# frankyeh/UNet-Studio

Hardware: AMD Instinct MI355X
Metric: voxels/sec 3D U-Net train step @128^3 bf16 (higher is better)
Workload: dtype bf16

## Files before the change

unet-studio_amd/csrc/kernels_direct.hip:

```cpp
#include "device_util.h"

namespace unet {

__global__ void k_pack_conv_w(const float* __restrict__ w, float* __restrict__ wf, float* __restrict__ wd, int Cin, int Cout,
                              int k3, int CoutP, int CinP) {
    int64_t i = (int64_t)blockIdx.x * blockDim.x + threadIdx.x;
    int64_t nf = (int64_t)k3 * Cin * CoutP, nd = (int64_t)k3 * Cout * CinP;
    if (i < nf) {
        int co = (int)(i % CoutP); int64_t r = i / CoutP;
        int ci = (int)(r % Cin); int t = (int)(r / Cin);
        wf[i] = co < Cout ? w[((int64_t)co * Cin + ci) * k3 + t] : 0.f;
    }
    if (i < nd) {
        int ci = (int)(i % CinP); int64_t r = i / CinP;
        int co = (int)(r % Cout); int t = (int)(r / Cout);
        wd[i] = ci < Cin ? w[((int64_t)co * Cin + ci) * k3 + t] : 0.f;
    }
}
__global__ void k_pack_convt_w(const float* __restrict__ w, float* __restrict__ wf, float* __restrict__ wd, int Cin, int Cout,
                               int CoutP, int CinP) {
    int64_t i = (int64_t)blockIdx.x * blockDim.x + threadIdx.x;
    int64_t nf = (int64_t)8 * Cin * CoutP, nd = (int64_t)8 * Cout * CinP;
    if (i < nf) {
        int co = (int)(i % CoutP); int64_t r = i / CoutP;
// ... 621 lines not shown
    small_wgrad_epilogue<NACC>(acc, nchunk, sm, a.slab + (int64_t)blockIdx.x * (O + Cout), [=](int ch, int i) {
        if (i < CO * 16) { int c = i / 16, k = i % 16; return c < Cout ? c * Cin + ch * 16 + k : -1; }
        int c = i - CO * 16;
        return (ch == 0 && c < Cout) ? O + c : -1;
    });
}

constexpr int FIRST_TY = 8;
template <typename T> __global__ void __launch_bounds__(256) k_wgrad_first(WgradRegArgs a) {
    extern __shared__ float sm[];
    constexpr int NACC = 27 * 4 + 4;
    const ConvGeom& g = a.g;
    const int nchunk = 1 << a.lc, chunk = threadIdx.x & (nchunk - 1), co0 = chunk * 4;
    const int W4 = g.W >> 2, WP = (g.W + 2 + 3) & ~3;
    const int ytiles = (g.H + FIRST_TY - 1) / FIRST_TY, tiles = g.D * ytiles;
    const int nin = 3 * (FIRST_TY + 2) * WP;
    const int items = (FIRST_TY * W4) << a.lc;
    const T* dy = (const T*)a.dy;
    float acc[NACC];
#pragma unroll
    for (int i = 0; i < NACC; ++i) acc[i] = 0.f;
    for (int tile = blockIdx.x; tile < tiles; tile += gridDim.x) {
        const int z = tile / ytiles, y0 = (tile % ytiles) * FIRST_TY;
        __syncthreads();
        for (int i = threadIdx.x; i < nin; i += 256) {
            const int px = i % WP, r = i / WP, ry = r % (FIRST_TY + 2), rz = r / (FIRST_TY + 2);
            const int iz = z + rz - 1, iy = y0 + ry - 1, ix = px - 1;
            float v = 0.f;
            if (iz >= 0 && iz < g.D && iy >= 0 && iy < g.H && ix >= 0 && ix < g.W) v = view_ld<T>(a.src, ((int64_t)iz * g.H + iy) * g.W + ix, 0);
            sm[i] = v;
        }
        __syncthreads();
        for (int it = threadIdx.x; it < items; it += 256) {
            const int run = it >> a.lc, ty = run / W4, x0 = (run % W4) * 4;
            if (y0 + ty >= g.H) continue;
            float in[3][3][6], ds[4][4];
#pragma unroll
            for (int kz = 0; kz < 3; ++kz)
#pragma unroll
                for (int ky = 0; ky < 3; ++ky) {
                    const float* row = sm + (kz * (FIRST_TY + 2) + ty + ky) * WP + x0;
                    const float4 q = *(const float4*)row;
                    const float2 q2 = *(const float2*)(row + 4);
                    in[kz][ky][0] = q.x; in[kz][ky][1] = q.y; in[kz][ky][2] = q.z; in[kz][ky][3] = q.w;
                    in[kz][ky][4] = q2.x; in[kz][ky][5] = q2.y;
                }
            const int64_t vox = ((int64_t)z * g.H + y0 + ty) * g.W + x0;
#pragma unroll
            for (int u = 0; u < 4; ++u) {
                if constexpr (sizeof(T) == 2) {
                    const uint2 r = *(const uint2*)((const bf16*)dy + (vox + u) * g.Cout + co0);
                    ds[u][0] = __uint_as_float(r.x << 16); ds[u][1] = __uint_as_float(r.x & 0xffff0000u);
                    ds[u][2] = __uint_as_float(r.y << 16); ds[u][3] = __uint_as_float(r.y & 0xffff0000u);
                } else {
                    const float4 r = *(const float4*)((const float*)dy + (vox + u) * g.Cout + co0);
                    ds[u][0] = r.x; ds[u][1] = r.y; ds[u][2] = r.z; ds[u][3] = r.w;
                }
            }
#pragma unroll
            for (int kz = 0; kz < 3; ++kz)
#pragma unroll
                for (int ky = 0; ky < 3; ++ky)
#pragma unroll
                    for (int kx = 0; kx < 3; ++kx)
#pragma unroll
                        for (int u = 0; u < 4; ++u)
#pragma unroll
                            for (int c = 0; c < 4; ++c)
                                acc[((kz * 3 + ky) * 3 + kx) * 4 + c] = fmaf(in[kz][ky][u + kx], ds[u][c], acc[((kz * 3 + ky) * 3 + kx) * 4 + c]);
#pragma unroll
            for (int u = 0; u < 4; ++u)
#pragma unroll
                for (int c = 0; c < 4; ++c) acc[108 + c] += ds[u][c];
        }
    }
    __syncthreads();
    const int Cout = g.Cout, O = 27 * Cout;
    small_wgrad_epilogue<NACC>(acc, nchunk, sm, a.slab + (int64_t)blockIdx.x * (O + Cout), [=](int ch, int i) {
        if (i < 108) return (ch * 4 + i % 4) * 27 + i / 4;
        return O + ch * 4 + (i - 108);
    });
}

template <typename T> __device__ __forceinline__ void load_chunk16(const SrcDesc& src, bool plain, int64_t v, int c0, bool ok, float (&x)[16],
                                                                  const float* ss = nullptr, int Cin = 0) {
    if constexpr (sizeof(T) == 2) {
        if (plain || ss) {
            uint4 r0 = make_uint4(0, 0, 0, 0), r1 = r0;
            if (ok) {
                const uint4* q = (const uint4*)((const bf16*)src.ptr + v * src.C + c0);
                r0 = q[0]; r1 = q[1];
            }
            const unsigned w[8] = {r0.x, r0.y, r0.z, r0.w, r1.x, r1.y, r1.z, r1.w};
#pragma unroll
            for (int k = 0; k < 8; ++k) { x[2 * k] = __uint_as_float(w[k] << 16); x[2 * k + 1] = __uint_as_float(w[k] & 0xffff0000u); }
            if (!plain) {
#pragma unroll
                for (int k4 = 0; k4 < 4; ++k4) {
                    const float4 sc = *(const float4*)(ss + c0 + 4 * k4), sh = *(const float4*)(ss + Cin + c0 + 4 * k4);
                    x[4 * k4] = act_f(x[4 * k4] * sc.x + sh.x, src.act); x[4 * k4 + 1] = act_f(x[4 * k4 + 1] * sc.y + sh.y, src.act);
                    x[4 * k4 + 2] = act_f(x[4 * k4 + 2] * sc.z + sh.z, src.act); x[4 * k4 + 3] = act_f(x[4 * k4 + 3] * sc.w + sh.w, src.act);
                }
                if (!ok) {
#pragma unroll
                    for (int k = 0; k < 16; ++k) x[k] = 0.f;
                }
            }
            return;
        }
    }
#pragma unroll
    for (int k = 0; k < 16; ++k) x[k] = ok ? view_ld<T>(src, v, c0 + k) : 0.f;
}
template <typename T> __device__ __forceinline__ const float* stage_view(const SrcDesc& src, float* sm_after_filter, int Cin) {
    if (sizeof(T) != 2 || !src.scale) return nullptr;
    for (int i = threadIdx.x; i < Cin; i += 256) { sm_after_filter[i] = src.scale[i]; sm_after_filter[Cin + i] = src.shift[i]; }
    return sm_after_filter;
}

struct HeadArgs {
    SrcDesc src;
    const float* w;
    const float* bias;
    int Cin, Cout, lc;
    int64_t S;
    void* y;
    float* out;
    const float* dy_planes;
    const void* dy_cl;
    DstGrad dst;
    float* slab;
};

template <typename T, int CO> __global__ void __launch_bounds__(256) k_head_fwd(HeadArgs a) {
    extern __shared__ float sm[];
    for (int i = threadIdx.x; i < CO * a.Cin; i += 256) sm[i] = i < a.Cout * a.Cin ? a.w[i] : 0.f;
    const float* ss = stage_view<T>(a.src, sm + CO * a.Cin, a.Cin);
    __syncthreads();
    const int nchunk = 1 << a.lc, chunk = threadIdx.x & (nchunk - 1), c0 = chunk * 16;
    const int64_t vstride = ((int64_t)gridDim.x * 256) >> a.lc;
    const bool plain = !a.src.scale && a.src.act == 0;
    float b[CO];
#pragma unroll
    for (int c = 0; c < CO; ++c) b[c] = (a.bias && c < a.Cout) ? a.bias[c] : 0.f;
    for (int64_t v0 = ((int64_t)blockIdx.x * 256 + threadIdx.x) >> a.lc; v0 < ((a.S + 63) & ~(int64_t)63); v0 += vstride) {
        const bool ok = v0 < a.S;
        float x[16], o[CO];
        load_chunk16<T>(a.src, plain, v0, c0, ok, x, ss, a.Cin);
#pragma unroll
        for (int c = 0; c < CO; ++c) {
            const float4* wr = (const float4*)(sm + c * a.Cin + c0);
            float r = 0.f;
#pragma unroll
            for (int k4 = 0; k4 < 4; ++k4) {
                const float4 w4 = wr[k4];
                r = fmaf(x[4 * k4], w4.x, r); r = fmaf(x[4 * k4 + 1], w4.y, r); r = fmaf(x[4 * k4 + 2], w4.z, r); r = fmaf(x[4 * k4 + 3], w4.w, r);
            }
            for (int m = 1; m < nchunk; m <<= 1) r += __shfl_xor(r, m);
            o[c] = r + b[c];
        }
        if (ok && chunk == 0) {
#pragma unroll
            for (int c = 0; c < CO; ++c) {
                if (c < a.Cout) {
                    if (a.out) a.out[(int64_t)c * a.S + v0] = o[c];
                    if (a.y) st<T>((T*)a.y, v0 * a.Cout + c, o[c]);
                }
            }
        }
    }
}

template <typename T, int CO> __global__ void __launch_bounds__(256) k_head_bwd(HeadArgs a) {
    extern __shared__ float sm[];
    constexpr int NACC = CO * 16 + CO;
    for (int i = threadIdx.x; i < CO * a.Cin; i += 256) sm[i] = i < a.Cout * a.Cin ? a.w[i] : 0.f;
    const float* ss = stage_view<T>(a.src, sm + CO * a.Cin, a.Cin);
    __syncthreads();
    const int nchunk = 1 << a.lc, chunk = threadIdx.x & (nchunk - 1), c0 = chunk * 16;
    const int64_t vstride = ((int64_t)gridDim.x * 256) >> a.lc;
    const bool plain = !a.src.scale && a.src.act == 0;
    float acc[NACC];
#pragma unroll
    for (int i = 0; i < NACC; ++i) acc[i] = 0.f;
    auto fetch = [&](int64_t v, float (&xo)[16], float (&dout)[CO]) {
        load_chunk16<T>(a.src, plain, v, c0, true, xo, ss, a.Cin);
#pragma unroll
        for (int c = 0; c < CO; ++c) {
            dout[c] = 0.f;
            if (c < a.Cout) dout[c] = a.dy_planes ? a.dy_planes[(int64_t)c * a.S + v] : ld<T>((const T*)a.dy_cl, v * a.Cout + c);
        }
    };
    float xn[16], dn[CO];
    int64_t v0 = ((int64_t)blockIdx.x * 256 + threadIdx.x) >> a.lc;
    if (v0 < a.S) fetch(v0, xn, dn);
    for (; v0 < a.S; v0 += vstride) {
        float x[16], d[CO];
#pragma unroll
        for (int k = 0; k < 16; ++k) x[k] = xn[k];
#pragma unroll
        for (int c = 0; c < CO; ++c) d[c] = dn[c];
        if (v0 + vstride < a.S) fetch(v0 + vstride, xn, dn);
        if (a.slab) {
#pragma unroll
            for (int c = 0; c < CO; ++c) {
#pragma unroll
                for (int k = 0; k < 16; ++k) acc[c * 16 + k] = fmaf(d[c], x[k], acc[c * 16 + k]);
                acc[CO * 16 + c] += d[c];
            }
        }
        if (a.dst.ptr) {
            float g[16];
#pragma unroll
            for (int k = 0; k < 16; ++k) g[k] = 0.f;
#pragma unroll
            for (int c = 0; c < CO; ++c) {
                const float4* wr = (const float4*)(sm + c * a.Cin + c0);
#pragma unroll
                for (int k4 = 0; k4 < 4; ++k4) {
                    const float4 w4 = wr[k4];
                    g[4 * k4] = fmaf(d[c], w4.x, g[4 * k4]); g[4 * k4 + 1] = fmaf(d[c], w4.y, g[4 * k4 + 1]);
                    g[4 * k4 + 2] = fmaf(d[c], w4.z, g[4 * k4 + 2]); g[4 * k4 + 3] = fmaf(d[c], w4.w, g[4 * k4 + 3]);
                }
            }
            if constexpr (sizeof(T) == 2) {
                uint4* q = (uint4*)((bf16*)a.dst.ptr + v0 * a.dst.C + c0);
                if (a.dst.accumulate) {
                    const uint4 r0 = q[0], r1 = q[1];
                    const unsigned w[8] = {r0.x, r0.y, r0.z, r0.w, r1.x, r1.y, r1.z, r1.w};
#pragma unroll
                    for (int k = 0; k < 8; ++k) { g[2 * k] += __uint_as_float(w[k] << 16); g[2 * k + 1] += __uint_as_float(w[k] & 0xffff0000u); }
                }
                unsigned pk[8];
#pragma unroll
                for (int k = 0; k < 8; ++k) {
                    const bf16 lo = __float2bfloat16(g[2 * k]), hi = __float2bfloat16(g[2 * k + 1]);
                    pk[k] = (unsigned)__builtin_bit_cast(unsigned short, lo) | ((unsigned)__builtin_bit_cast(unsigned short, hi) << 16);
                }
                q[0] = make_uint4(pk[0], pk[1], pk[2], pk[3]); q[1] = make_uint4(pk[4], pk[5], pk[6], pk[7]);
            } else {
                float* q = (float*)a.dst.ptr + v0 * a.dst.C + c0;
#pragma unroll
                for (int k = 0; k < 16; ++k) q[k] = a.dst.accumulate ? q[k] + g[k] : g[k];
            }
        }
    }
    if (a.slab) {
        __syncthreads();
        const int Cin = a.Cin, Cout = a.Cout, O = Cin * Cout;
        small_wgrad_epilogue<NACC>(acc, nchunk, sm, a.slab + (int64_t)blockIdx.x * (O + Cout), [=](int ch, int i) {
            if (i < CO * 16) { int c = i / 16, k = i % 16; return c < Cout ? c * Cin + ch * 16 + k : -1; }
            int c = i - CO * 16;
            return (ch == 0 && c < Cout) ? O + c : -1;
        });
    }
}

static int ilog2_exact(int v) { int l = 0; while ((1 << l) < v) ++l; return (1 << l) == v ? l : -1; }
static bool wgrad_head_ok(const ConvGeom& g, int nsrc) {
    return nsrc == 1 && g.ks == 1 && g.stride == 1 && g.Cout <= 8 && g.Cin % 16 == 0 && ilog2_exact(g.Cin / 16) >= 0 && g.Cin <= 256;
}
static bool wgrad_first_ok(const ConvGeom& g, int nsrc) {
    return nsrc == 1 && g.ks == 3 && g.stride == 1 && g.Cin == 1 && g.Cout % 4 == 0 && ilog2_exact(g.Cout / 4) >= 0 && g.Cout <= 64 &&
           g.W % 4 == 0 && g.W <= 256;
}
static int wgrad_reg_blocks(int64_t items4) { int64_t nb = (items4 + 1023) / 1024; return nb < 1 ? 1 : (nb > 512 ? 512 : (int)nb); }
static bool wgrad_rows_ok(const ConvGeom& g) {
    int k3 = g.ks * g.ks * g.ks;
    int WI = (g.Wo - 1) * g.stride + g.ks;
    size_t lds = ((size_t)g.ks * g.ks * WI * g.Cin + (size_t)g.Wo * g.Cout) * 4;
    return (int64_t)k3 * g.Cin * g.Cout <= 1024 && lds <= 48 * 1024;
}

static int wgrad_small_blocks(const ConvGeom& g) { int rows = g.Do * g.Ho; return rows < 1024 ? rows : 1024; }
bool wgrad_small_supported(const ConvGeom& g, int nsrc) { return wgrad_head_ok(g, nsrc) || wgrad_first_ok(g, nsrc) || wgrad_rows_ok(g); }
size_t wgrad_small_scratch_bytes(const ConvGeom& g) {
    int k3 = g.ks * g.ks * g.ks;
    int64_t So = (int64_t)g.Do * g.Ho * g.Wo;
    size_t O = (size_t)k3 * g.Cin * g.Cout;
    size_t rows = (size_t)wgrad_small_blocks(g) * O * 4 + bias_grad_scratch_bytes(g.Cout, So) + 256;
    size_t regs = (size_t)512 * (O + g.Cout) * 4 + 256;
    return rows > regs ? rows : regs;
}
void launch_conv_wgrad_small(int dtype, const ConvGeom& g, const SrcDesc* src, int nsrc, const void* dy, float* dw, float* db,
                             void* scratch, hipStream_t s) {
    const int k3 = g.ks * g.ks * g.ks;
    const int64_t O = (int64_t)k3 * g.Cin * g.Cout;
    const bool head = wgrad_head_ok(g, nsrc), first = !head && wgrad_first_ok(g, nsrc);
    if (head || first) {
        WgradRegArgs a;
        a.g = g; a.src = src[0]; a.dy = dy; a.slab = (float*)scratch;
        const int64_t S = (int64_t)g.D * g.H * g.W;
        int nb;
        if (head) {
            a.lc = ilog2_exact(g.Cin / 16);
            nb = wgrad_reg_blocks((S << a.lc) * 4);
            const int CO = g.Cout <= 2 ? 2 : g.Cout <= 4 ? 4 : g.Cout <= 6 ? 6 : 8;
            const size_t lds = small_wgrad_lds_bytes(CO * 17, 1 << a.lc);
            switch (CO) {
                case 2: UNET_DISPATCH(dtype, (k_wgrad_head<T, 2><<<nb, 256, lds, s>>>(a))); break;
                case 4: UNET_DISPATCH(dtype, (k_wgrad_head<T, 4><<<nb, 256, lds, s>>>(a))); break;
                case 6: UNET_DISPATCH(dtype, (k_wgrad_head<T, 6><<<nb, 256, lds, s>>>(a))); break;
                default: UNET_DISPATCH(dtype, (k_wgrad_head<T, 8><<<nb, 256, lds, s>>>(a))); break;
            }
        } else {
            a.lc = ilog2_exact(g.Cout / 4);
            const int tiles = g.D * ((g.H + FIRST_TY - 1) / FIRST_TY);
            nb = tiles < 512 ? tiles : 512;
            const size_t l0 = (size_t)3 * (FIRST_TY + 2) * ((g.W + 5) & ~3) * 4, l1 = small_wgrad_lds_bytes(112, 1 << a.lc);
            const size_t lds = l0 > l1 ? l0 : l1;
            UNET_DISPATCH(dtype, (k_wgrad_first<T><<<nb, 256, lds, s>>>(a)));
        }
        slab_reduce2(a.slab, nb, O + g.Cout, dw, O, db, s);
        return;
    }
    WgradSmallArgs a;
    a.g = g; a.nsrc = nsrc; a.src[0] = src[0]; if (nsrc > 1) a.src[1] = src[1];
    a.dy = dy; a.slab = (float*)scratch;
    int nb = wgrad_small_blocks(g);
    int WI = (g.Wo - 1) * g.stride + g.ks;
    size_t lds = ((size_t)g.ks * g.ks * WI * g.Cin + (size_t)g.Wo * g.Cout) * 4;
    UNET_DISPATCH(dtype, (k_wgrad_small<T><<<nb, 256, lds, s>>>(a)));
    slab_reduce(a.slab, nb, O, dw, s);
    if (db) launch_bias_grad(dtype, dy, g.Cout, (int64_t)g.Do * g.Ho * g.Wo, db, (float*)scratch + (size_t)nb * O, s);
}

bool head_supported(const ConvGeom& g, int nsrc) { return wgrad_head_ok(g, nsrc); }
size_t head_bwd_scratch_bytes(const ConvGeom& g) { return (size_t)512 * ((size_t)g.Cin * g.Cout + g.Cout) * 4 + 256; }
template <typename T> static void head_launch(bool bwd, int CO, int nb, size_t lds, const HeadArgs& a, hipStream_t s) {
    switch (CO) {
        case 2: if (bwd) k_head_bwd<T, 2><<<nb, 256, lds, s>>>(a); else k_head_fwd<T, 2><<<nb, 256, lds, s>>>(a); break;
        case 4: if (bwd) k_head_bwd<T, 4><<<nb, 256, lds, s>>>(a); else k_head_fwd<T, 4><<<nb, 256, lds, s>>>(a); break;
        case 6: if (bwd) k_head_bwd<T, 6><<<nb, 256, lds, s>>>(a); else k_head_fwd<T, 6><<<nb, 256, lds, s>>>(a); break;
        default: if (bwd) k_head_bwd<T, 8><<<nb, 256, lds, s>>>(a); else k_head_fwd<T, 8><<<nb, 256, lds, s>>>(a); break;
    }
}
static int head_co(int Cout) { return Cout <= 2 ? 2 : Cout <= 4 ? 4 : Cout <= 6 ? 6 : 8; }
void launch_head_fwd(int dtype, const ConvGeom& g, const SrcDesc& src, const float* w, const float* bias, void* y, float* out_ncdhw,
                     hipStream_t s) {
    HeadArgs a = {};
    a.src = src; a.w = w; a.bias = bias; a.Cin = g.Cin; a.Cout = g.Cout; a.lc = ilog2_exact(g.Cin / 16);
    a.S = (int64_t)g.D * g.H * g.W; a.y = y; a.out = out_ncdhw;
    const int CO = head_co(g.Cout);
    int64_t items = ((a.S + 63) & ~(int64_t)63) << a.lc;
    int64_t nb = (items + 255) / 256;
    if (nb > 2048) nb = 2048;
    UNET_DISPATCH(dtype, (head_launch<T>(false, CO, (int)nb, (size_t)(CO + 2) * g.Cin * 4, a, s)));
}
void launch_head_bwd(int dtype, const ConvGeom& g, const SrcDesc& src, const float* dy_ncdhw, const void* dy_cl, const float* w,
                     DstGrad dst, float* dw, float* db, void* scratch, hipStream_t s, bool defer_reduce) {
    HeadArgs a = {};
    a.src = src; a.w = w; a.Cin = g.Cin; a.Cout = g.Cout; a.lc = ilog2_exact(g.Cin / 16);
    a.S = (int64_t)g.D * g.H * g.W; a.dy_planes = dy_ncdhw; a.dy_cl = dy_cl; a.dst = dst;
    a.slab = dw ? (float*)scratch : nullptr;
    const int CO = head_co(g.Cout);
    const int nb = wgrad_reg_blocks((a.S << a.lc) * 4);
    const size_t l0 = (size_t)(CO + 2) * g.Cin * 4, l1 = small_wgrad_lds_bytes(CO * 17, 1 << a.lc);
    UNET_DISPATCH(dtype, (head_launch<T>(true, CO, nb, l0 > l1 ? l0 : l1, a, s)));
    if (dw && !defer_reduce) slab_reduce2(a.slab, nb, (int64_t)g.Cin * g.Cout + g.Cout, dw, (int64_t)g.Cin * g.Cout, db, s);
}
void launch_head_bwd_reduce(const ConvGeom& g, float* dw, float* db, const void* scratch, hipStream_t s) {
    const int lc = ilog2_exact(g.Cin / 16);
    const int nb = wgrad_reg_blocks((((int64_t)g.D * g.H * g.W) << lc) * 4);
    slab_reduce2((const float*)scratch, nb, (int64_t)g.Cin * g.Cout + g.Cout, dw, (int64_t)g.Cin * g.Cout, db, s);
}

}
```

unet-studio_amd/csrc/kernels_elem.hip:

```cpp
#include "device_util.h"
#include "sgd_update.h"

namespace unet {

template <typename T> __global__ void k_pack_input(const float* __restrict__ x, T* __restrict__ y, int C, int64_t S) {
    int64_t i = (int64_t)blockIdx.x * 256 + threadIdx.x;
    if (i >= S * C) return;
    int c = (int)(i % C); int64_t v = i / C;
    st<T>(y, i, x[(int64_t)c * S + v]);
}
void launch_pack_input(int dtype, const float* x, void* y, int C, int64_t S, hipStream_t s) {
    UNET_DISPATCH(dtype, (k_pack_input<T><<<cdiv64(S * C, 256), 256, 0, s>>>(x, (T*)y, C, S)));
}

template <typename T> __global__ void k_export(SrcDesc src, float* __restrict__ y, int64_t S) {
    int64_t i = (int64_t)blockIdx.x * 256 + threadIdx.x;
    if (i >= S * src.C) return;
    int c = (int)(i / S); int64_t v = i % S;
    y[i] = view_ld<T>(src, v, c);
}
void launch_export(int dtype, SrcDesc src, float* y, int64_t S, hipStream_t s) {
    UNET_DISPATCH(dtype, (k_export<T><<<cdiv64(S * src.C, 256), 256, 0, s>>>(src, y, S)));
}
void launch_unpack_ncdhw(int dtype, const void* g, float* out, int C, int64_t S, hipStream_t s) {
// ... 717 lines not shown
        bool valid = t < C;
        if (!valid) continue;
        int tt = k ? (int)(t - k + 1 > 0 ? t - k + 1 : 0) : (int)t;
        VoxelLogits L = make_vl(logits, S, v, k);
        float mx = -INFINITY;
        for (int c = 0; c < oc; ++c) mx = fmaxf(mx, L.get(c));
        float sum = 0.f;
        for (int c = 0; c < oc; ++c) sum += __expf(L.get(c) - mx);
        float inv = 1.f / sum, psq = 0.f, pt = 0.f;
        for (int c = 0; c < oc; ++c) {
            float p = clamp_p(__expf(L.get(c) - mx) * inv);
            psq = fmaf(p, p, psq);
            if (c == tt) pt = p;
            if (c >= 1) atomicAdd(&sh[3 + oc + c], p + (c == tt ? 1.f : 0.f));
        }
        if (tt >= 1) atomicAdd(&sh[3 + tt], pt);
        ce += -(L.get(tt) - mx - __logf(sum));
        mse += psq - 2.f * pt + 1.f;
        nv += 1.f;
    }
    atomicAdd(&sh[0], ce); atomicAdd(&sh[1], mse); atomicAdd(&sh[2], nv);
    __syncthreads();
    for (int i = threadIdx.x; i < np; i += 256) partial[(int64_t)blockIdx.x * np + i] = sh[i];
}
template <int OCMAX>
__global__ void __launch_bounds__(256) k_loss_partial_reg(const float* __restrict__ logits, const int64_t* __restrict__ target, int C,
                                                          int64_t S, int k, float* __restrict__ partial) {
    constexpr int RS = 3 + 2 * OCMAX + 1;
    __shared__ float red[4 * RS];
    const int oc = k ? C - k + 1 : C, np = 3 + 2 * oc;
    float ce = 0.f, mse = 0.f, nv = 0.f, inter[OCMAX], card[OCMAX];
#pragma unroll
    for (int c = 0; c < OCMAX; ++c) { inter[c] = 0.f; card[c] = 0.f; }
    for (int64_t v = (int64_t)blockIdx.x * 256 + threadIdx.x; v < S; v += (int64_t)gridDim.x * 256) {
        int64_t t = target[v];
        if (!(t < C)) continue;
        int tt = k ? (int)(t - k + 1 > 0 ? t - k + 1 : 0) : (int)t;
        VoxelLogits L = make_vl(logits, S, v, k);
        float lg[OCMAX], mx = -INFINITY;
#pragma unroll
        for (int c = 0; c < OCMAX; ++c) { lg[c] = c < oc ? L.get(c) : -INFINITY; mx = fmaxf(mx, lg[c]); }
        float sum = 0.f;
#pragma unroll
        for (int c = 0; c < OCMAX; ++c) { lg[c] = c < oc ? __expf(lg[c] - mx) : 0.f; sum += lg[c]; }
        float inv = 1.f / sum, psq = 0.f, pt = 0.f, lt = 0.f;
#pragma unroll
        for (int c = 0; c < OCMAX; ++c) {
            if (c < oc) {
                float p = clamp_p(lg[c] * inv);
                psq = fmaf(p, p, psq);
                bool hit = c == tt;
                if (hit) { pt = p; lt = L.get(c); inter[c] += p; }
                card[c] += p + (hit ? 1.f : 0.f);
            }
        }
        ce += -(lt - mx - __logf(sum));
        mse += psq - 2.f * pt + 1.f;
        nv += 1.f;
    }
    auto wsum = [](float v) { for (int o = 32; o > 0; o >>= 1) v += __shfl_xor(v, o); return v; };
    const int lane = threadIdx.x & 63, wave = threadIdx.x >> 6;
    float w3[3] = {wsum(ce), wsum(mse), wsum(nv)};
    if (lane == 0) { red[wave * RS + 0] = w3[0]; red[wave * RS + 1] = w3[1]; red[wave * RS + 2] = w3[2]; }
#pragma unroll
    for (int c = 0; c < OCMAX; ++c) {
        if (c < oc) {
            const float a = wsum(inter[c]), b = wsum(card[c]);
            if (lane == 0) { red[wave * RS + 3 + c] = a; red[wave * RS + 3 + oc + c] = b; }
        }
    }
    __syncthreads();
    if ((int)threadIdx.x < np)
        partial[(int64_t)blockIdx.x * np + threadIdx.x] = red[threadIdx.x] + red[RS + threadIdx.x] + red[2 * RS + threadIdx.x] + red[3 * RS + threadIdx.x];
}
template <int OCMAX>
__global__ void __launch_bounds__(256) k_loss_partial_v4(const float* __restrict__ logits, const int64_t* __restrict__ target, int C,
                                                         int64_t S, float* __restrict__ partial) {
    constexpr int RS = 3 + 2 * OCMAX + 1;
    __shared__ float red[4 * RS];
    const int oc = C, np = 3 + 2 * oc;
    float ce = 0.f, mse = 0.f, nv = 0.f, inter[OCMAX], card[OCMAX];
#pragma unroll
    for (int c = 0; c < OCMAX; ++c) { inter[c] = 0.f; card[c] = 0.f; }
    const int64_t S4 = S >> 2;
    for (int64_t q4 = (int64_t)blockIdx.x * 256 + threadIdx.x; q4 < S4; q4 += (int64_t)gridDim.x * 256) {
        const longlong2 t01 = ((const longlong2*)target)[2 * q4], t23 = ((const longlong2*)target)[2 * q4 + 1];
        const int64_t tv[4] = {t01.x, t01.y, t23.x, t23.y};
        float4 pl[OCMAX];
#pragma unroll
        for (int c = 0; c < OCMAX; ++c)
            pl[c] = c < oc ? ((const float4*)(logits + (int64_t)c * S))[q4] : make_float4(-INFINITY, -INFINITY, -INFINITY, -INFINITY);
#pragma unroll
        for (int j = 0; j < 4; ++j) {
            const int64_t t = tv[j];
            if (!(t < C)) continue;
            const int tt = (int)t;
            float lg[OCMAX], mx = -INFINITY;
#pragma unroll
            for (int c = 0; c < OCMAX; ++c) { lg[c] = j == 0 ? pl[c].x : j == 1 ? pl[c].y : j == 2 ? pl[c].z : pl[c].w; mx = fmaxf(mx, lg[c]); }
            float sum = 0.f, lt = 0.f;
#pragma unroll
            for (int c = 0; c < OCMAX; ++c) { if (c == tt) lt = lg[c]; lg[c] = c < oc ? __expf(lg[c] - mx) : 0.f; sum += lg[c]; }
            const float inv = 1.f / sum;
            float psq = 0.f, pt = 0.f;
#pragma unroll
            for (int c = 0; c < OCMAX; ++c) {
                if (c < oc) {
                    const float p = clamp_p(lg[c] * inv);
                    psq = fmaf(p, p, psq);
                    const bool hit = c == tt;
                    if (hit) { pt = p; inter[c] += p; }
                    card[c] += p + (hit ? 1.f : 0.f);
                }
            }
            ce += -(lt - mx - __logf(sum));
            mse += psq - 2.f * pt + 1.f;
            nv += 1.f;
        }
    }
    auto wsum = [](float v) { for (int o = 32; o > 0; o >>= 1) v += __shfl_xor(v, o); return v; };
    const int lane = threadIdx.x & 63, wave = threadIdx.x >> 6;
    float w3[3] = {wsum(ce), wsum(mse), wsum(nv)};
    if (lane == 0) { red[wave * RS + 0] = w3[0]; red[wave * RS + 1] = w3[1]; red[wave * RS + 2] = w3[2]; }
#pragma unroll
    for (int c = 0; c < OCMAX; ++c) {
        if (c < oc) {
            const float a = wsum(inter[c]), b = wsum(card[c]);
            if (lane == 0) { red[wave * RS + 3 + c] = a; red[wave * RS + 3 + oc + c] = b; }
        }
    }
    __syncthreads();
    if ((int)threadIdx.x < np)
        partial[(int64_t)blockIdx.x * np + threadIdx.x] = red[threadIdx.x] + red[RS + threadIdx.x] + red[2 * RS + threadIdx.x] + red[3 * RS + threadIdx.x];
}
static inline bool loss_v4_ok(const void* a, const void* b, const void* c, int C, int64_t S, int collapse) {
    return !collapse && C <= 8 && S % 4 == 0 && S >= 4096 && ((uintptr_t)a | (uintptr_t)b | (uintptr_t)c) % 16 == 0;
}
void launch_loss_partial(const float* logits, const int64_t* target, int C, int64_t S, int collapse, float* partial, hipStream_t s) {
    int oc = collapse ? C - collapse + 1 : C;
    if (loss_v4_ok(logits, target, nullptr, C, S, collapse)) {
        k_loss_partial_v4<8><<<loss_blocks(S), 256, 0, s>>>(logits, target, C, S, partial);
        return;
    }
    if (oc <= 8) k_loss_partial_reg<8><<<loss_blocks(S), 256, 0, s>>>(logits, target, C, S, collapse, partial);
    else if (oc <= 32) k_loss_partial_reg<32><<<loss_blocks(S), 256, 0, s>>>(logits, target, C, S, collapse, partial);
    else k_loss_partial<<<loss_blocks(S), 256, (3 + 2 * oc) * sizeof(float), s>>>(logits, target, C, S, collapse, partial);
}

__global__ void __launch_bounds__(1024) k_loss_finalize(const float* __restrict__ partial, int nblk, int oc, float weight, int cost_mask,
                                                       float* level_out, float* totals, int set_stats) {
    extern __shared__ double shd[];
    int np = 3 + 2 * oc;
    const int wv = threadIdx.x >> 6, ln = threadIdx.x & 63;
    for (int i = wv; i < np; i += (int)(blockDim.x >> 6)) {
        double a = 0.0;
        for (int b = ln; b < nblk; b += 64) a += partial[(int64_t)b * np + i];
        for (int o = 32; o > 0; o >>= 1) a += __shfl_down(a, o);
        if (ln == 0) shd[i] = a;
    }
    __syncthreads();
    if (threadIdx.x == 0) {
        double n = shd[2] < 1.0 ? 1.0 : shd[2];
        double eps = (double)1e-5f, dsum = 0.0;
        for (int c = 1; c < oc; ++c) dsum += (2.0 * shd[3 + c] + eps) / (shd[3 + oc + c] + eps);
        double ce = shd[0] / n, mse = shd[1] / n, dice = 1.0 - dsum / (double)(oc - 1 > 1 ? oc - 1 : 1);
        level_out[0] = (float)ce; level_out[1] = (float)dice; level_out[2] = (float)mse; level_out[3] = (float)n;
        for (int c = 0; c < oc; ++c) { level_out[4 + c] = (float)shd[3 + c]; level_out[4 + oc + c] = (float)shd[3 + oc + c]; }
        double sel = 0.0;
        if (!(cost_mask & 7)) sel = ce;
        else sel = ((cost_mask & 1) ? ce : 0.0) + ((cost_mask & 2) ? dice : 0.0) + ((cost_mask & 4) ? mse : 0.0);
        totals[0] += (float)(weight * sel);
        if (set_stats) { totals[1] = (float)ce; totals[2] = (float)dice; totals[3] = (float)mse; }
    }
}
void launch_loss_finalize(const float* partial, int nblk, int oc, float weight, int cost_mask, float* level_out, float* totals,
                          int set_stats, hipStream_t s) {
    k_loss_finalize<<<1, 3 + 2 * oc > 8 ? 1024 : 512, (3 + 2 * oc) * sizeof(double), s>>>(partial, nblk, oc, weight, cost_mask, level_out, totals, set_stats);
}

__global__ void __launch_bounds__(256) k_loss_grad(const float* __restrict__ logits, const int64_t* __restrict__ target, int C, int64_t S,
                                                   int k, const float* __restrict__ level_out, float weight, int cost_mask,
                                                   float* __restrict__ dlogits) {
    int oc = k ? C - k + 1 : C;
    int64_t v = (int64_t)blockIdx.x * 256 + threadIdx.x;
    if (v >= S) return;
    int64_t t = target[v];
    if (!(t < C)) {
        for (int c = 0; c < C; ++c) dlogits[(int64_t)c * S + v] = 0.f;
        return;
    }
    float w_ce = (!(cost_mask & 7) || (cost_mask & 1)) ? weight : 0.f;
    float w_dice = (cost_mask & 2) ? weight : 0.f, w_mse = (cost_mask & 4) ? weight : 0.f;
    float n = level_out[3];
    const float* inter = level_out + 4;
    const float* card = level_out + 4 + oc;
    float dden = (float)(oc - 1 > 1 ? oc - 1 : 1), eps = 1e-5f;
    int tt = k ? (int)(t - k + 1 > 0 ? t - k + 1 : 0) : (int)t;
    VoxelLogits L = make_vl(logits, S, v, k);
    float mx = -INFINITY;
    for (int c = 0; c < oc; ++c) mx = fmaxf(mx, L.get(c));
    float sum = 0.f;
    for (int c = 0; c < oc; ++c) sum += __expf(L.get(c) - mx);
    float inv = 1.f / sum;
    float dot = 0.f;
    for (int c = 0; c < oc; ++c) {
        float q = __expf(L.get(c) - mx) * inv, p = clamp_p(q), g = 0.f;
        g += w_mse * (2.f * p - (c == tt ? 2.f : 0.f)) / n;
        if (c >= 1) {
            float m = c == tt ? 1.f : 0.f, den = card[c] + eps;
            g += w_dice * (-(2.f * m * den - (2.f * inter[c] + eps)) / (den * den)) / dden;
        }
        if (!(q >= 1e-6f && q <= 1.0f - 1e-6f)) g = 0.f;
        dot = fmaf(g, q, dot);
    }
    float d0 = 0.f;
    for (int c = 0; c < oc; ++c) {
        float q = __expf(L.get(c) - mx) * inv, p = clamp_p(q), g = 0.f;
        g += w_mse * (2.f * p - (c == tt ? 2.f : 0.f)) / n;
        if (c >= 1) {
            float m = c == tt ? 1.f : 0.f, den = card[c] + eps;
            g += w_dice * (-(2.f * m * den - (2.f * inter[c] + eps)) / (den * den)) / dden;
        }
        if (!(q >= 1e-6f && q <= 1.0f - 1e-6f)) g = 0.f;
        float dl = q * (g - dot) + w_ce * (q - (c == tt ? 1.f : 0.f)) / n;
        if (k && c == 0) d0 = dl;
        else dlogits[(int64_t)(k ? c + k - 1 : c) * S + v] = dl;
    }
    if (k) {
        float m0 = -INFINITY;
        for (int c = 0; c < k; ++c) m0 = fmaxf(m0, logits[(int64_t)c * S + v]);
        float s0 = 0.f;
        for (int c = 0; c < k; ++c) s0 += __expf(logits[(int64_t)c * S + v] - m0);
        for (int c = 0; c < k; ++c) dlogits[(int64_t)c * S + v] = d0 * __expf(logits[(int64_t)c * S + v] - m0) / s0;
    }
}
template <int OCMAX>
__global__ void __launch_bounds__(256) k_loss_grad_v4(const float* __restrict__ logits, const int64_t* __restrict__ target, int C, int64_t S,
                                                      const float* __restrict__ level_out, float weight, int cost_mask,
                                                      float* __restrict__ dlogits) {
    const int oc = C;
    const int64_t q4 = (int64_t)blockIdx.x * 256 + threadIdx.x;
    if (q4 >= (S >> 2)) return;
    const float w_ce = (!(cost_mask & 7) || (cost_mask & 1)) ? weight : 0.f;
    const float w_dice = (cost_mask & 2) ? weight : 0.f, w_mse = (cost_mask & 4) ? weight : 0.f;
    const float n = level_out[3];
    const float dden = (float)(oc - 1 > 1 ? oc - 1 : 1), eps = 1e-5f;
    float dice_hit[OCMAX], dice_miss[OCMAX];
#pragma unroll
    for (int c = 0; c < OCMAX; ++c) {
        dice_hit[c] = dice_miss[c] = 0.f;
        if (c >= 1 && c < oc) {
            const float den = level_out[4 + oc + c] + eps, in2 = 2.f * level_out[4 + c] + eps;
            dice_hit[c] = w_dice * (-(2.f * 1.f * den - in2) / (den * den)) / dden;
            dice_miss[c] = w_dice * (-(2.f * 0.f * den - in2) / (den * den)) / dden;
        }
    }
    const longlong2 t01 = ((const longlong2*)target)[2 * q4], t23 = ((const longlong2*)target)[2 * q4 + 1];
    const int64_t tv[4] = {t01.x, t01.y, t23.x, t23.y};
    float4 pl[OCMAX];
#pragma unroll
    for (int c = 0; c < OCMAX; ++c)
        pl[c] = c < oc ? ((const float4*)(logits + (int64_t)c * S))[q4] : make_float4(-INFINITY, -INFINITY, -INFINITY, -INFINITY);
    float out[OCMAX][4];
#pragma unroll
    for (int j = 0; j < 4; ++j) {
        const int64_t t = tv[j];
        const bool valid = t < C;
        const int tt = (int)t;
        float lg[OCMAX], mx = -INFINITY;
#pragma unroll
        for (int c = 0; c < OCMAX; ++c) { lg[c] = j == 0 ? pl[c].x : j == 1 ? pl[c].y : j == 2 ? pl[c].z : pl[c].w; mx = fmaxf(mx, lg[c]); }
        float sum = 0.f;
#pragma unroll
        for (int c = 0; c < OCMAX; ++c) { lg[c] = c < oc ? __expf(lg[c] - mx) : 0.f; sum += lg[c]; }
        const float inv = 1.f / sum;
        float g[OCMAX], dot = 0.f;
#pragma unroll
        for (int c = 0; c < OCMAX; ++c) {
            g[c] = 0.f;
            if (c < oc) {
                const float q = lg[c] * inv, p = clamp_p(q);
                float gg = 0.f;
                gg += w_mse * (2.f * p - (c == tt ? 2.f : 0.f)) / n;
                if (c >= 1) gg += c == tt ? dice_hit[c] : dice_miss[c];
                if (!(q >= 1e-6f && q <= 1.0f - 1e-6f)) gg = 0.f;
                dot = fmaf(gg, q, dot);
                g[c] = gg; lg[c] = q;
            }
        }
#pragma unroll
        for (int c = 0; c < OCMAX; ++c)
            out[c][j] = (c < oc && valid) ? lg[c] * (g[c] - dot) + w_ce * (lg[c] - (c == tt ? 1.f : 0.f)) / n : 0.f;
    }
#pragma unroll
    for (int c = 0; c < OCMAX; ++c)
        if (c < oc) ((float4*)(dlogits + (int64_t)c * S))[q4] = make_float4(out[c][0], out[c][1], out[c][2], out[c][3]);
}
void launch_loss_grad(const float* logits, const int64_t* target, int C, int64_t S, int collapse, const float* level_out, float weight,
                      int cost_mask, float* dlogits, hipStream_t s) {
    if (loss_v4_ok(logits, target, dlogits, C, S, collapse)) {
        k_loss_grad_v4<8><<<cdiv64(S >> 2, 256), 256, 0, s>>>(logits, target, C, S, level_out, weight, cost_mask, dlogits);
        return;
    }
    k_loss_grad<<<cdiv64(S, 256), 256, 0, s>>>(logits, target, C, S, collapse, level_out, weight, cost_mask, dlogits);
}

struct SumBufs { const float* in[UNET_SUM_MAX_BUFFERS]; int n; };
__global__ void __launch_bounds__(256) k_sum_buffers(SumBufs b, float* __restrict__ out, int64_t count, int zero_inputs) {
    for (int64_t i0 = ((int64_t)blockIdx.x * 256 + threadIdx.x) * 4; i0 < count; i0 += (int64_t)gridDim.x * 1024) {
        if (i0 + 3 < count) {
            float4 acc = *(const float4*)(b.in[0] + i0);
            for (int k = 1; k < b.n; ++k) {
                const float4 v = *(const float4*)(b.in[k] + i0);
                acc.x += v.x; acc.y += v.y; acc.z += v.z; acc.w += v.w;
            }
            *(float4*)(out + i0) = acc;
            if (zero_inputs)
                for (int k = 0; k < b.n; ++k)
                    if (b.in[k] != out) *(float4*)(const_cast<float*>(b.in[k]) + i0) = make_float4(0.f, 0.f, 0.f, 0.f);
        } else {
            for (int j = 0; j < 4 && i0 + j < count; ++j) {
                float acc = b.in[0][i0 + j];
                for (int k = 1; k < b.n; ++k) acc += b.in[k][i0 + j];
                out[i0 + j] = acc;
                if (zero_inputs)
                    for (int k = 0; k < b.n; ++k)
                        if (b.in[k] != out) const_cast<float*>(b.in[k])[i0 + j] = 0.f;
            }
        }
    }
}
void launch_sum_buffers(const float* const* bufs, int n, float* out, int64_t count, int zero_inputs, hipStream_t s) {
    SumBufs b;
    b.n = n;
    for (int k = 0; k < UNET_SUM_MAX_BUFFERS; ++k) b.in[k] = k < n ? bufs[k] : nullptr;
    int64_t nb = (count + 1023) / 1024;
    if (nb > 4096) nb = 4096;
    k_sum_buffers<<<(unsigned)nb, 256, 0, s>>>(b, out, count, zero_inputs);
}

__global__ void __launch_bounds__(256) k_sumsq_partial(const float* __restrict__ g, int64_t n, float scale, float* __restrict__ partial) {
    __shared__ double red[256];
    double acc = 0.0;
    for (int64_t i0 = ((int64_t)blockIdx.x * 256 + threadIdx.x) * 4; i0 < n; i0 += (int64_t)gridDim.x * 1024) {
        float r = 0.f;
        if (i0 + 3 < n) {
            const float4 v = *(const float4*)(g + i0);
            const float a0 = v.x * scale, a1 = v.y * scale, a2 = v.z * scale, a3 = v.w * scale;
            r = fmaf(a0, a0, fmaf(a1, a1, fmaf(a2, a2, a3 * a3)));
        } else {
            for (int j = 0; j < 4; ++j)
                if (i0 + j < n) { float x = g[i0 + j] * scale; r = fmaf(x, x, r); }
        }
        acc += (double)r;
    }
    red[threadIdx.x] = acc;
    __syncthreads();
    for (int o = 128; o > 0; o >>= 1) {
        if ((int)threadIdx.x < o) red[threadIdx.x] += red[threadIdx.x + o];
        __syncthreads();
    }
    if (threadIdx.x == 0) partial[blockIdx.x] = (float)red[0];
}
void launch_sumsq_partial(const float* g, int64_t n, float scale, float* partial, int nblk, hipStream_t s) {
    k_sumsq_partial<<<nblk, 256, 0, s>>>(g, n, scale, partial);
}

constexpr int SGD_MAXSEG = 1024;
__global__ void __launch_bounds__(256) k_sgd(float* __restrict__ p, float* __restrict__ g, float* __restrict__ m, int64_t n,
                                             const SgdSeg* __restrict__ segs, int nseg, const float* __restrict__ partial, int nblk,
                                             float lr, float momentum, int nesterov, float wdecay, float clip_norm, float grad_scale, float* norm_out) {
    __shared__ double red[256];
    __shared__ float s_coef;
    __shared__ int64_t s_off[SGD_MAXSEG];
    __shared__ float s_wd[SGD_MAXSEG];
    const int ns = nseg < SGD_MAXSEG ? nseg : SGD_MAXSEG;
    for (int k = threadIdx.x; k < ns; k += 256) { s_off[k] = segs[k].offset; s_wd[k] = segs[k].wd; }
    const SgdUpdate upd{sgd_clip_coef(partial, nblk, clip_norm, norm_out, red, &s_coef) * grad_scale, lr, momentum, nesterov};
    auto seg_of = [&](int64_t i) {
        int lo = 0, hi = nseg - 1;
        while (lo < hi) {
            int mid = (lo + hi + 1) >> 1;
            int64_t off = mid < SGD_MAXSEG ? s_off[mid] : segs[mid].offset;
            if (off <= i) lo = mid; else hi = mid - 1;
// ... 32 lines not shown
```

Before: 813.3 million.

## Add prefetching head fwd/bwd kernels and pair loss-kernel loads

Adds a new 1x1 head forward kernel for Cin=16 bf16 that processes four voxels per thread with vectorized float4 output stores. Adds a new head backward kernel that double-buffers the bf16 input and dy loads two strides ahead and specializes on the activation type. The loss partial and loss grad kernels now fetch two items before computing so more loads are in flight, and loss partial gets a 6-class instantiation. The goal is to hide memory latency in these small bandwidth-bound kernels, at the cost of more registers and extra template variants.

```diff
diff --git a/unet-studio_amd/csrc/kernels_direct.hip b/unet-studio_amd/csrc/kernels_direct.hip
--- a/unet-studio_amd/csrc/kernels_direct.hip
+++ b/unet-studio_amd/csrc/kernels_direct.hip
@@ -727,6 +727,23 @@
     });
 }
 
+__device__ __forceinline__ void unpack_chunk16(const uint4& r0, const uint4& r1, float (&x)[16]) {
+    const unsigned w[8] = {r0.x, r0.y, r0.z, r0.w, r1.x, r1.y, r1.z, r1.w};
+#pragma unroll
+    for (int k = 0; k < 8; ++k) { x[2 * k] = __uint_as_float(w[k] << 16); x[2 * k + 1] = __uint_as_float(w[k] & 0xffff0000u); }
+}
+__device__ __forceinline__ void view_chunk4(float (&x)[16], int k4, const float4 sc, const float4 sh, int act) {
+    x[4 * k4] = act_f(x[4 * k4] * sc.x + sh.x, act); x[4 * k4 + 1] = act_f(x[4 * k4 + 1] * sc.y + sh.y, act);
+    x[4 * k4 + 2] = act_f(x[4 * k4 + 2] * sc.z + sh.z, act); x[4 * k4 + 3] = act_f(x[4 * k4 + 3] * sc.w + sh.w, act);
+}
+__device__ __forceinline__ void expand_chunk16(const uint4& r0, const uint4& r1, bool plain, const float* ss, int c0, int Cin, int act,
+                                               float (&x)[16]) {
+    unpack_chunk16(r0, r1, x);
+    if (!plain) {
+#pragma unroll
+        for (int k4 = 0; k4 < 4; ++k4) view_chunk4(x, k4, *(const float4*)(ss + c0 + 4 * k4), *(const float4*)(ss + Cin + c0 + 4 * k4), act);
+    }
+}
 template <typename T> __device__ __forceinline__ void load_chunk16(const SrcDesc& src, bool plain, int64_t v, int c0, bool ok, float (&x)[16],
                                                                   const float* ss = nullptr, int Cin = 0) {
     if constexpr (sizeof(T) == 2) {
@@ -736,16 +753,8 @@
                 const uint4* q = (const uint4*)((const bf16*)src.ptr + v * src.C + c0);
                 r0 = q[0]; r1 = q[1];
             }
-            const unsigned w[8] = {r0.x, r0.y, r0.z, r0.w, r1.x, r1.y, r1.z, r1.w};
-#pragma unroll
-            for (int k = 0; k < 8; ++k) { x[2 * k] = __uint_as_float(w[k] << 16); x[2 * k + 1] = __uint_as_float(w[k] & 0xffff0000u); }
+            expand_chunk16(r0, r1, plain, ss, c0, Cin, src.act, x);
             if (!plain) {
-#pragma unroll
-                for (int k4 = 0; k4 < 4; ++k4) {
-                    const float4 sc = *(const float4*)(ss + c0 + 4 * k4), sh = *(const float4*)(ss + Cin + c0 + 4 * k4);
-                    x[4 * k4] = act_f(x[4 * k4] * sc.x + sh.x, src.act); x[4 * k4 + 1] = act_f(x[4 * k4 + 1] * sc.y + sh.y, src.act);
-                    x[4 * k4 + 2] = act_f(x[4 * k4 + 2] * sc.z + sh.z, src.act); x[4 * k4 + 3] = act_f(x[4 * k4 + 3] * sc.w + sh.w, src.act);
-                }
                 if (!ok) {
 #pragma unroll
                     for (int k = 0; k < 16; ++k) x[k] = 0.f;
@@ -816,6 +825,69 @@
     }
 }
 
+template <int ACT> __device__ __forceinline__ void view_voxels4(float (&x)[4][16], const float* ss) {
+#pragma unroll
+    for (int k4 = 0; k4 < 4; ++k4) {
+        asm volatile("" ::: "memory");
+        const float4 sc = *(const float4*)(ss + 4 * k4), sh = *(const float4*)(ss + 16 + 4 * k4);
+#pragma unroll
+        for (int j = 0; j < 4; ++j) view_chunk4(x[j], k4, sc, sh, ACT);
+    }
+}
+template <int CO> __global__ void __launch_bounds__(256) k_head_fwd_v4(HeadArgs a) {
+    extern __shared__ float sm[];
+    for (int i = threadIdx.x; i < CO * 16; i += 256) sm[i] = i < a.Cout * 16 ? a.w[i] : 0.f;
+    const float* ss = stage_view<bf16>(a.src, sm + CO * 16, 16);
+    __syncthreads();
+    float b[CO];
+#pragma unroll
+    for (int c = 0; c < CO; ++c) b[c] = (a.bias && c < a.Cout) ? a.bias[c] : 0.f;
+    const int64_t S4 = a.S >> 2, G = (int64_t)gridDim.x * 256;
+    auto fetch = [&](int64_t q4, uint4 (&r)[8]) {
+#pragma unroll
+        for (int j = 0; j < 4; ++j) {
+            const uint4* q = (const uint4*)((const bf16*)a.src.ptr + (4 * q4 + j) * a.src.C);
+            r[2 * j] = q[0]; r[2 * j + 1] = q[1];
+        }
+    };
+    for (int64_t q4 = (int64_t)blockIdx.x * 256 + threadIdx.x; q4 < S4; q4 += G) {
+        uint4 r[8];
+        fetch(q4, r);
+        float x[4][16];
+#pragma unroll
+        for (int j = 0; j < 4; ++j) unpack_chunk16(r[2 * j], r[2 * j + 1], x[j]);
+        if (ss) {
+            if (a.src.act == 2) view_voxels4<2>(x, ss);
+            else if (a.src.act == 1) view_voxels4<1>(x, ss);
+            else view_voxels4<0>(x, ss);
+        }
+#pragma unroll
+        for (int c = 0; c < CO; ++c) {
+            asm volatile("" ::: "memory");
+            __builtin_amdgcn_sched_barrier(0);
+            const float4* wr = (const float4*)(sm + c * 16);
+            float acc[4] = {0.f, 0.f, 0.f, 0.f};
+#pragma unroll
+            for (int k4 = 0; k4 < 4; ++k4) {
+                const float4 w4 = wr[k4];
+#pragma unroll
+                for (int j = 0; j < 4; ++j) {
+                    float t = acc[j];
+                    t = fmaf(x[j][4 * k4], w4.x, t); t = fmaf(x[j][4 * k4 + 1], w4.y, t); t = fmaf(x[j][4 * k4 + 2], w4.z, t); t = fmaf(x[j][4 * k4 + 3], w4.w, t);
+                    acc[j] = t;
+                }
+            }
+            if (c < a.Cout)
+                ((float4*)(a.out + (int64_t)c * a.S))[q4] = make_float4(acc[0] + b[c], acc[1] + b[c], acc[2] + b[c], acc[3] + b[c]);
+        }
+    }
+}
+static bool head_fwd_v4_ok(int dtype, const HeadArgs& a) {
+    const bool vec = a.src.scale ? a.src.act <= 2 : a.src.act == 0;
+    return dtype != 0 && a.Cin == 16 && a.S % 4 == 0 && vec && a.out && !a.y && a.src.C % 8 == 0 &&
+           ((uintptr_t)a.src.ptr | (uintptr_t)a.out) % 16 == 0;
+}
+
 template <typename T, int CO> __global__ void __launch_bounds__(256) k_head_bwd(HeadArgs a) {
     extern __shared__ float sm[];
     constexpr int NACC = CO * 16 + CO;
@@ -899,6 +971,101 @@
             return (ch == 0 && c < Cout) ? O + c : -1;
         });
     }
+}
+
+template <int CO, int ACT> __global__ void __launch_bounds__(256) k_head_bwd2(HeadArgs a) {
+    extern __shared__ float sm[];
+    constexpr int NACC = CO * 16 + CO;
+    struct Held { uint4 r0, r1; float d[CO]; };
+    for (int i = threadIdx.x; i < CO * a.Cin; i += 256) sm[i] = i < a.Cout * a.Cin ? a.w[i] : 0.f;
+    const float* ss = stage_view<bf16>(a.src, sm + CO * a.Cin, a.Cin);
+    __syncthreads();
+    const int nchunk = 1 << a.lc, chunk = threadIdx.x & (nchunk - 1), c0 = chunk * 16;
+    const int64_t vstride = ((int64_t)gridDim.x * 256) >> a.lc;
+    float acc[NACC];
+#pragma unroll
+    for (int i = 0; i < NACC; ++i) acc[i] = 0.f;
+    auto fetch = [&](int64_t v, Held& h) {
+        const uint4* q = (const uint4*)((const bf16*)a.src.ptr + v * a.src.C + c0);
+        h.r0 = q[0]; h.r1 = q[1];
+#pragma unroll
+        for (int c = 0; c < CO; ++c) h.d[c] = a.dy_planes[(int64_t)(c < a.Cout ? c : 0) * a.S + v];
+    };
+    auto step = [&](int64_t v, Held& h) {
+        asm volatile("" ::: "memory");
+        uint4* q = (uint4*)((bf16*)a.dst.ptr + v * a.dst.C + c0);
+        uint4 old0 = make_uint4(0, 0, 0, 0), old1 = old0;
+        if (a.dst.ptr && a.dst.accumulate) { old0 = q[0]; old1 = q[1]; }
+        float x[16], d[CO];
+        unpack_chunk16(h.r0, h.r1, x);
+#pragma unroll
+        for (int c = 0; c < CO; ++c) {
+            asm volatile("v_mov_b32 %0, %1" : "=v"(d[c]) : "v"(h.d[c]));
+            d[c] = c < a.Cout ? d[c] : 0.f;
+        }
+        fetch(v + 2 * vstride < a.S ? v + 2 * vstride : a.S - 1, h);
+        if (ss) {
+#pragma unroll
+            for (int k4 = 0; k4 < 4; ++k4) view_chunk4(x, k4, *(const float4*)(ss + c0 + 4 * k4), *(const float4*)(ss + a.Cin + c0 + 4 * k4), ACT);
+        }
+        if (a.slab) {
+#pragma unroll
+            for (int c = 0; c < CO; ++c) {
+#pragma unroll
+                for (int k = 0; k < 16; ++k) acc[c * 16 + k] = fmaf(d[c], x[k], acc[c * 16 + k]);
+                acc[CO * 16 + c] += d[c];
+            }
+        }
+        if (a.dst.ptr) {
+            float g[16];
+#pragma unroll
+            for (int k = 0; k < 16; ++k) g[k] = 0.f;
+#pragma unroll
+            for (int c = 0; c < CO; ++c) {
+                __builtin_amdgcn_sched_barrier(0);
+                const float4* wr = (const float4*)(sm + c * a.Cin + c0);
+#pragma unroll
+                for (int k4 = 0; k4 < 4; ++k4) {
+                    const float4 w4 = wr[k4];
+                    g[4 * k4] = fmaf(d[c], w4.x, g[4 * k4]); g[4 * k4 + 1] = fmaf(d[c], w4.y, g[4 * k4 + 1]);
+                    g[4 * k4 + 2] = fmaf(d[c], w4.z, g[4 * k4 + 2]); g[4 * k4 + 3] = fmaf(d[c], w4.w, g[4 * k4 + 3]);
+                }
+            }
+            if (a.dst.accumulate) {
+                const unsigned w[8] = {old0.x, old0.y, old0.z, old0.w, old1.x, old1.y, old1.z, old1.w};
+#pragma unroll
+                for (int k = 0; k < 8; ++k) { g[2 * k] += __uint_as_float(w[k] << 16); g[2 * k + 1] += __uint_as_float(w[k] & 0xffff0000u); }
+            }
+            unsigned pk[8];
+#pragma unroll
+            for (int k = 0; k < 8; ++k) {
+                const bf16 lo = __float2bfloat16(g[2 * k]), hi = __float2bfloat16(g[2 * k + 1]);
+                pk[k] = (unsigned)__builtin_bit_cast(unsigned short, lo) | ((unsigned)__builtin_bit_cast(unsigned short, hi) << 16);
+            }
+            q[0] = make_uint4(pk[0], pk[1], pk[2], pk[3]); q[1] = make_uint4(pk[4], pk[5], pk[6], pk[7]);
+        }
+    };
+    Held ha, hb;
+    int64_t v0 = ((int64_t)blockIdx.x * 256 + threadIdx.x) >> a.lc;
+    fetch(v0 < a.S ? v0 : a.S - 1, ha);
+    fetch(v0 + vstride < a.S ? v0 + vstride : a.S - 1, hb);
+    for (; v0 + vstride < a.S; v0 += 2 * vstride) {
+        step(v0, ha);
+        step(v0 + vstride, hb);
+    }
+    if (v0 < a.S) step(v0, ha);
+    if (a.slab) {
+        __syncthreads();
+        const int Cin = a.Cin, Cout = a.Cout, O = Cin * Cout;
+        small_wgrad_epilogue<NACC>(acc, nchunk, sm, a.slab + (int64_t)blockIdx.x * (O + Cout), [=](int ch, int i) {
+            if (i < CO * 16) { int c = i / 16, k = i % 16; return c < Cout ? c * Cin + ch * 16 + k : -1; }
+            int c = i - CO * 16;
+            return (ch == 0 && c < Cout) ? O + c : -1;
+        });
+    }
+}
+static bool head_bwd2_ok(int dtype, const HeadArgs& a) {
+    return dtype != 0 && a.dy_planes && (a.src.scale ? a.src.act <= 2 : a.src.act == 0);
 }
 
 static int ilog2_exact(int v) { int l = 0; while ((1 << l) < v) ++l; return (1 << l) == v ? l : -1; }
@@ -980,6 +1147,19 @@
         default: if (bwd) k_head_bwd<T, 8><<<nb, 256, lds, s>>>(a); else k_head_fwd<T, 8><<<nb, 256, lds, s>>>(a); break;
     }
 }
+template <int ACT> static void head_bwd2_launch_act(int CO, int nb, size_t lds, const HeadArgs& a, hipStream_t s) {
+    switch (CO) {
+        case 2: k_head_bwd2<2, ACT><<<nb, 256, lds, s>>>(a); break;
+        case 4: k_head_bwd2<4, ACT><<<nb, 256, lds, s>>>(a); break;
+        case 6: k_head_bwd2<6, ACT><<<nb, 256, lds, s>>>(a); break;
+        default: k_head_bwd2<8, ACT><<<nb, 256, lds, s>>>(a); break;
+    }
+}
+static void head_bwd2_launch(int CO, int act, int nb, size_t lds, const HeadArgs& a, hipStream_t s) {
+    if (act == 2) head_bwd2_launch_act<2>(CO, nb, lds, a, s);
+    else if (act == 1) head_bwd2_launch_act<1>(CO, nb, lds, a, s);
+    else head_bwd2_launch_act<0>(CO, nb, lds, a, s);
+}
 static int head_co(int Cout) { return Cout <= 2 ? 2 : Cout <= 4 ? 4 : Cout <= 6 ? 6 : 8; }
 void launch_head_fwd(int dtype, const ConvGeom& g, const SrcDesc& src, const float* w, const float* bias, void* y, float* out_ncdhw,
                      hipStream_t s) {
@@ -987,6 +1167,18 @@
     a.src = src; a.w = w; a.bias = bias; a.Cin = g.Cin; a.Cout = g.Cout; a.lc = ilog2_exact(g.Cin / 16);
     a.S = (int64_t)g.D * g.H * g.W; a.y = y; a.out = out_ncdhw;
     const int CO = head_co(g.Cout);
+    if (head_fwd_v4_ok(dtype, a)) {
+        int64_t nb4 = ((a.S >> 2) + 255) / 256;
+        if (nb4 > 2048) nb4 = 2048;
+        const size_t lds = (size_t)(CO + 2) * 16 * 4;
+        switch (CO) {
+            case 2: k_head_fwd_v4<2><<<(int)nb4, 256, lds, s>>>(a); break;
+            case 4: k_head_fwd_v4<4><<<(int)nb4, 256, lds, s>>>(a); break;
+            case 6: k_head_fwd_v4<6><<<(int)nb4, 256, lds, s>>>(a); break;
+            default: k_head_fwd_v4<8><<<(int)nb4, 256, lds, s>>>(a); break;
+        }
+        return;
+    }
     int64_t items = ((a.S + 63) & ~(int64_t)63) << a.lc;
     int64_t nb = (items + 255) / 256;
     if (nb > 2048) nb = 2048;
@@ -1001,7 +1193,8 @@
     const int CO = head_co(g.Cout);
     const int nb = wgrad_reg_blocks((a.S << a.lc) * 4);
     const size_t l0 = (size_t)(CO + 2) * g.Cin * 4, l1 = small_wgrad_lds_bytes(CO * 17, 1 << a.lc);
-    UNET_DISPATCH(dtype, (head_launch<T>(true, CO, nb, l0 > l1 ? l0 : l1, a, s)));
+    if (head_bwd2_ok(dtype, a)) head_bwd2_launch(CO, a.src.scale ? a.src.act : 0, nb, l0 > l1 ? l0 : l1, a, s);
+    else UNET_DISPATCH(dtype, (head_launch<T>(true, CO, nb, l0 > l1 ? l0 : l1, a, s)));
     if (dw && !defer_reduce) slab_reduce2(a.slab, nb, (int64_t)g.Cin * g.Cout + g.Cout, dw, (int64_t)g.Cin * g.Cout, db, s);
 }
 void launch_head_bwd_reduce(const ConvGeom& g, float* dw, float* db, const void* scratch, hipStream_t s) {
diff --git a/unet-studio_amd/csrc/kernels_elem.hip b/unet-studio_amd/csrc/kernels_elem.hip
--- a/unet-studio_amd/csrc/kernels_elem.hip
+++ b/unet-studio_amd/csrc/kernels_elem.hip
@@ -823,14 +823,15 @@
     float ce = 0.f, mse = 0.f, nv = 0.f, inter[OCMAX], card[OCMAX];
 #pragma unroll
     for (int c = 0; c < OCMAX; ++c) { inter[c] = 0.f; card[c] = 0.f; }
-    const int64_t S4 = S >> 2;
-    for (int64_t q4 = (int64_t)blockIdx.x * 256 + threadIdx.x; q4 < S4; q4 += (int64_t)gridDim.x * 256) {
-        const longlong2 t01 = ((const longlong2*)target)[2 * q4], t23 = ((const longlong2*)target)[2 * q4 + 1];
-        const int64_t tv[4] = {t01.x, t01.y, t23.x, t23.y};
-        float4 pl[OCMAX];
+    const int64_t S4 = S >> 2, G = (int64_t)gridDim.x * 256;
+    auto fetch = [&](int64_t q4, longlong2 (&tq)[2], float4 (&pl)[OCMAX]) {
+        tq[0] = ((const longlong2*)target)[2 * q4]; tq[1] = ((const longlong2*)target)[2 * q4 + 1];
 #pragma unroll
         for (int c = 0; c < OCMAX; ++c)
             pl[c] = c < oc ? ((const float4*)(logits + (int64_t)c * S))[q4] : make_float4(-INFINITY, -INFINITY, -INFINITY, -INFINITY);
+    };
+    auto item = [&](const longlong2 (&tq)[2], const float4 (&pl)[OCMAX]) {
+        const int64_t tv[4] = {tq[0].x, tq[0].y, tq[1].x, tq[1].y};
 #pragma unroll
         for (int j = 0; j < 4; ++j) {
             const int64_t t = tv[j];
@@ -858,6 +859,16 @@
             mse += psq - 2.f * pt + 1.f;
             nv += 1.f;
         }
+    };
+    constexpr bool PAIR = OCMAX <= 6;
+    for (int64_t q4 = (int64_t)blockIdx.x * 256 + threadIdx.x; q4 < S4; q4 += PAIR ? 2 * G : G) {
+        const bool two = PAIR && q4 + G < S4;
+        longlong2 ta[2], tb[2];
+        float4 pa[OCMAX], pb[OCMAX];
+        fetch(q4, ta, pa);
+        fetch(two ? q4 + G : q4, tb, pb);
+        item(ta, pa);
+        if (two) item(tb, pb);
     }
     auto wsum = [](float v) { for (int o = 32; o > 0; o >>= 1) v += __shfl_xor(v, o); return v; };
     const int lane = threadIdx.x & 63, wave = threadIdx.x >> 6;
@@ -880,7 +891,8 @@
 void launch_loss_partial(const float* logits, const int64_t* target, int C, int64_t S, int collapse, float* partial, hipStream_t s) {
     int oc = collapse ? C - collapse + 1 : C;
     if (loss_v4_ok(logits, target, nullptr, C, S, collapse)) {
-        k_loss_partial_v4<8><<<loss_blocks(S), 256, 0, s>>>(logits, target, C, S, partial);
+        if (C <= 6) k_loss_partial_v4<6><<<loss_blocks(S), 256, 0, s>>>(logits, target, C, S, partial);
+        else k_loss_partial_v4<8><<<loss_blocks(S), 256, 0, s>>>(logits, target, C, S, partial);
         return;
     }
     if (oc <= 8) k_loss_partial_reg<8><<<loss_blocks(S), 256, 0, s>>>(logits, target, C, S, collapse, partial);
@@ -980,8 +992,9 @@
                                                       const float* __restrict__ level_out, float weight, int cost_mask,
                                                       float* __restrict__ dlogits) {
     const int oc = C;
-    const int64_t q4 = (int64_t)blockIdx.x * 256 + threadIdx.x;
-    if (q4 >= (S >> 2)) return;
+    const int64_t S4 = S >> 2, q4a = (int64_t)blockIdx.x * 256 + threadIdx.x, q4b = q4a + (int64_t)gridDim.x * 256;
+    if (q4a >= S4) return;
+    const bool two = q4b < S4;
     const float w_ce = (!(cost_mask & 7) || (cost_mask & 1)) ? weight : 0.f;
     const float w_dice = (cost_mask & 2) ? weight : 0.f, w_mse = (cost_mask & 4) ? weight : 0.f;
     const float n = level_out[3];
@@ -996,12 +1009,14 @@
             dice_miss[c] = w_dice * (-(2.f * 0.f * den - in2) / (den * den)) / dden;
         }
     }
-    const longlong2 t01 = ((const longlong2*)target)[2 * q4], t23 = ((const longlong2*)target)[2 * q4 + 1];
-    const int64_t tv[4] = {t01.x, t01.y, t23.x, t23.y};
-    float4 pl[OCMAX];
-#pragma unroll
-    for (int c = 0; c < OCMAX; ++c)
-        pl[c] = c < oc ? ((const float4*)(logits + (int64_t)c * S))[q4] : make_float4(-INFINITY, -INFINITY, -INFINITY, -INFINITY);
+    auto fetch = [&](int64_t q4, longlong2 (&tq)[2], float4 (&pl)[OCMAX]) {
+        tq[0] = ((const longlong2*)target)[2 * q4]; tq[1] = ((const longlong2*)target)[2 * q4 + 1];
+#pragma unroll
+        for (int c = 0; c < OCMAX; ++c)
+            pl[c] = c < oc ? ((const float4*)(logits + (int64_t)c * S))[q4] : make_float4(-INFINITY, -INFINITY, -INFINITY, -INFINITY);
+    };
+    auto item = [&](int64_t q4, const longlong2 (&tq)[2], const float4 (&pl)[OCMAX]) {
+    const int64_t tv[4] = {tq[0].x, tq[0].y, tq[1].x, tq[1].y};
     float out[OCMAX][4];
 #pragma unroll
     for (int j = 0; j < 4; ++j) {
@@ -1036,11 +1051,19 @@
 #pragma unroll
     for (int c = 0; c < OCMAX; ++c)
         if (c < oc) ((float4*)(dlogits + (int64_t)c * S))[q4] = make_float4(out[c][0], out[c][1], out[c][2], out[c][3]);
+    };
+    longlong2 ta[2], tb[2];
+    float4 pa[OCMAX], pb[OCMAX];
+    fetch(q4a, ta, pa);
+    fetch(two ? q4b : q4a, tb, pb);
+    item(q4a, ta, pa);
+    if (two) item(q4b, tb, pb);
 }
 void launch_loss_grad(const float* logits, const int64_t* target, int C, int64_t S, int collapse, const float* level_out, float weight,
                       int cost_mask, float* dlogits, hipStream_t s) {
     if (loss_v4_ok(logits, target, dlogits, C, S, collapse)) {
-        k_loss_grad_v4<8><<<cdiv64(S >> 2, 256), 256, 0, s>>>(logits, target, C, S, level_out, weight, cost_mask, dlogits);
+        const unsigned nb = cdiv64(S >> 2, 256);
+        k_loss_grad_v4<8><<<nb >= 2048 ? (nb + 1) / 2 : nb, 256, 0, s>>>(logits, target, C, S, level_out, weight, cost_mask, dlogits);
         return;
     }
     k_loss_grad<<<cdiv64(S, 256), 256, 0, s>>>(logits, target, C, S, collapse, level_out, weight, cost_mask, dlogits);
```

Measured after the change: 819.2 million (median of 6 runs). Within noise of the previous version (+0.7%).
